# colinvaz/nmf-toolbox

Hardware: AMD Instinct MI355X
Metric: NMF multiplicative-update iterations/s (higher is better)
Workload: dtype f32; 1 GPU; nmf.m kl MU, V=16384x65536 K=256 fp32, V column-sharded over 1 GPU(s); m=16384, n=65536, K=256, T=1, divergence=kl

## Files before the change

### nmf_toolbox_amd/build.py

```python
from __future__ import annotations

import os
import subprocess
import sys
from concurrent.futures import ThreadPoolExecutor

HERE = os.path.dirname(os.path.abspath(__file__))
CSRC = os.path.join(HERE, "csrc")
INC = os.path.join(os.path.dirname(HERE), "include")
OUT = os.path.join(HERE, "libnmfx.so")
SOURCES = ["fused_cnmf_a.hip", "fused_cnmf_b.hip", "fused_cnmf_c.hip", "fused_cnmf_e.hip", "fused_cnmf_d.hip", "fused_cnmf_g.hip", "fused_cnmf_f.hip", "gemm_pipe_edge.hip", "gemm_pipe.hip", "gemm.hip", "fused_k224_256.hip", "fused_rag_k224_256.hip", "fused_k128_192.hip", "fused_rag_k128_192.hip", "fused_k32_96.hip", "fused_rag_k32_96.hip", "fused.hip", "aux.hip", "projfunc.hip", "small_mm.hip", "gemm64.hip", "engine.hip", "host_io.hip", "blocking.hip", "sc.hip", "sc64.hip", "multi_sc.hip", "rccl_backend.hip", "cmfwisa.hip", "seminmf.hip", "nmf64.hip", "nmf_batch.hip", "cnmf_batch.hip", "wnmf.hip", "wcnmf.hip"]
ARCH = "gfx950"


def _torch_lib_dir():
    try:
        import importlib.util
        spec = importlib.util.find_spec("torch")
        if spec and spec.origin:
            d = os.path.join(os.path.dirname(spec.origin), "lib")
            if os.path.exists(os.path.join(d, "libamdhip64.so")):
                return d
    except Exception:
        pass
    return None


def _deps(src, incdirs, seen=None):
    import re
    seen = set() if seen is None else seen
    if src in seen or not os.path.exists(src):
        return seen
    seen.add(src)
    with open(src) as f:
        for name in re.findall(r'^\s*#\s*include\s*"([^"]+)"', f.read(), re.M):
            for d in [os.path.dirname(src)] + incdirs:
                cand = os.path.join(d, name)
                if os.path.exists(cand):
                    _deps(cand, incdirs, seen)
                    break
    return seen


def _newer(src_list, target):
    if not os.path.exists(target):
        return True
    t = os.path.getmtime(target)
    return any(os.path.getmtime(s) > t for s in src_list)


VARIANTS = {
    "r5": ["-DNMFX_KL_MODE=0", "-DNMFX_G2_VEC=0", "-DNMFX_G1_ASM=0"],
    "kl1": ["-DNMFX_KL_MODE=1", "-DNMFX_G2_VEC=0", "-DNMFX_G1_ASM=0"],
    "kl2": ["-DNMFX_KL_MODE=2", "-DNMFX_G2_VEC=0", "-DNMFX_G1_ASM=0"],
    "kl2g2": ["-DNMFX_KL_MODE=2", "-DNMFX_G2_VEC=1", "-DNMFX_G1_ASM=0"],
}


def build(force: bool = False, verbose: bool = False, sanitize: bool = False, variant: str = "") -> str:
    srcs = [os.path.join(CSRC, s) for s in SOURCES if os.path.exists(os.path.join(CSRC, s))]
    objdir = os.path.join(CSRC, "_obj_asan" if sanitize else ("_obj_" + variant if variant else "_obj"))
    out = os.path.join(HERE, "libnmfx_asan.so") if sanitize else (os.path.join(HERE, "libnmfx_%s.so" % variant) if variant else OUT)
    vdefs = VARIANTS[variant] if variant else []
    san = ["-fsanitize=address,undefined", "-fno-sanitize=function", "-fno-gpu-sanitize", "-fno-sanitize-recover=undefined", "-Xarch_host", "-g", "-Xarch_host", "-fno-omit-frame-pointer"] if sanitize else []
    os.makedirs(objdir, exist_ok=True)
    hipcc = os.environ.get("HIPCC", "/opt/rocm/bin/hipcc")

    def compile_one(src):
        obj = os.path.join(objdir, os.path.basename(src) + ".o")
        if force or _newer(sorted(_deps(src, [CSRC, INC])) + [os.path.abspath(__file__)], obj):
            cmd = [hipcc, f"--offload-arch={ARCH}", "-O3", "-std=c++17", "-fPIC", "-Wall", "-Werror=uninitialized", "-Wno-pass-failed"] + san + vdefs + [
                   "-I", INC, "-I", CSRC, "-c", src, "-o", obj]
            if os.path.basename(src).startswith("fused_"):
                cmd[3:3] = ["-mllvm", "-pragma-unroll-threshold=1000000"]
            if verbose:
                print(" ".join(cmd), flush=True)
            subprocess.check_call(cmd)
        return obj

    with ThreadPoolExecutor(max_workers=min(len(srcs), 8)) as ex:
        objs = list(ex.map(compile_one, srcs))
    if force or _newer(objs, out):
        tl = _torch_lib_dir()
        libdirs = ([tl] if tl else []) + ["/opt/rocm/lib"]
        if sanitize:
            cmd = ["/opt/rocm/lib/llvm/bin/clang++", "-shared", "-fsanitize=address,undefined", "-fno-sanitize=function", "-o", out] + objs
        else:
            cmd = ["g++", "-shared", "-o", out] + objs
# ... 34 lines not shown
```

### nmf_toolbox_amd/csrc/fused.hip

```cpp
#include "nmfx_internal.h"

namespace nmfx {

bool fused_supported(int K) { return K >= 32 && K <= 256 && K % 32 == 0; }
bool fused_supported_T(int Kh, int T) {
    static const int ok[][2] = {{64, 8}, {64, 4}, {32, 8}, {32, 16}, {64, 2}, {32, 4}, {128, 2}, {128, 4},
                                {32, 3}, {32, 5}, {32, 6}, {64, 3}, {32, 10}, {32, 12}, {64, 5}, {64, 6},
                                {32, 7}, {32, 9}, {32, 11}, {64, 7}, {32, 13}, {32, 14}, {32, 15}, {128, 3}, {256, 2}};
    for (const auto &c : ok) if (c[0] == Kh && c[1] == T) return true;
    return false;
}

bool fused_supported_T_dual(int Kh, int T) { return fused_supported_T(Kh, T); }

#define NMFX_DECL(name) nmfx_status name(hipStream_t st, const FusedParams &p, int nsplit, bool d_rc, int func, bool do_g2, int epi)
NMFX_DECL(launch_fused_k32_96); NMFX_DECL(launch_fused_k128_192); NMFX_DECL(launch_fused_k224_256);
NMFX_DECL(launch_fused_rag_k32_96); NMFX_DECL(launch_fused_rag_k128_192); NMFX_DECL(launch_fused_rag_k224_256);
#undef NMFX_DECL
#define NMFX_DECL_T(name) nmfx_status name(hipStream_t st, const FusedParams &p, int nsplit, int func, bool do_g2)
NMFX_DECL_T(launch_fused_cnmf_a); NMFX_DECL_T(launch_fused_cnmf_b); NMFX_DECL_T(launch_fused_cnmf_c); NMFX_DECL_T(launch_fused_cnmf_d); NMFX_DECL_T(launch_fused_cnmf_e); NMFX_DECL_T(launch_fused_cnmf_f); NMFX_DECL_T(launch_fused_cnmf_g);
#undef NMFX_DECL_T

nmfx_status launch_fused(hipStream_t st, const FusedParams &p, int nsplit, bool d_rc, int func, bool do_g2, int epi) {
    constexpr int FT_ROWS = 128, FT_C = 64;
    if (p.R <= 0 || p.Cn <= 0 || p.c_per_split % FT_C || p.c_per_split <= 0 || nsplit < 1 || (long)(nsplit - 1) * p.c_per_split >= p.Cn) {
        set_error("launch_fused: bad split (R=%ld Cn=%ld c_per_split=%ld nsplit=%d)", p.R, p.Cn, p.c_per_split, nsplit);
        return NMFX_ERR_INVALID;
    }
    if (p.T > 1) {
        if (!d_rc || epi != 0 || p.K % p.T != 0 || !fused_supported_T(p.K / p.T, p.T)) {
            set_error("launch_fused: cnmf pass with (K = %d, T = %d) is not instantiated", p.K, p.T);
            return NMFX_ERR_UNSUPPORTED;
        }
        const int kh = p.K / p.T;
        if ((kh == 64 && (p.T == 8 || p.T == 4))) return launch_fused_cnmf_a(st, p, nsplit, func, do_g2);
        if (kh == 32 && (p.T == 8 || p.T == 16)) return launch_fused_cnmf_b(st, p, nsplit, func, do_g2);
        if ((kh == 32 && (p.T == 3 || p.T == 5 || p.T == 6)) || (kh == 64 && p.T == 3)) return launch_fused_cnmf_d(st, p, nsplit, func, do_g2);
        if ((kh == 32 && (p.T == 10 || p.T == 12)) || (kh == 64 && (p.T == 5 || p.T == 6))) return launch_fused_cnmf_e(st, p, nsplit, func, do_g2);
        if ((kh == 32 && (p.T == 7 || p.T == 9 || p.T == 11)) || (kh == 64 && p.T == 7)) return launch_fused_cnmf_f(st, p, nsplit, func, do_g2);
        if ((kh == 32 && (p.T == 13 || p.T == 14 || p.T == 15)) || (kh == 128 && p.T == 3) || (kh == 256 && p.T == 2)) return launch_fused_cnmf_g(st, p, nsplit, func, do_g2);
        return launch_fused_cnmf_c(st, p, nsplit, func, do_g2);
    }
    if (!fused_supported(p.K)) { set_error("launch_fused: K=%d not supported (multiples of 32 up to 256)", p.K); return NMFX_ERR_UNSUPPORTED; }
    if (d_rc && do_g2 && func == 0 && epi == 0 && p.os_k == 1 && p.os_r != 1 && NMFX_G2_VEC) epi = 2;
    const bool rag = p.R % FT_ROWS != 0 || p.Cn % FT_C != 0;
    if (p.K <= 96) return rag ? launch_fused_rag_k32_96(st, p, nsplit, d_rc, func, do_g2, epi) : launch_fused_k32_96(st, p, nsplit, d_rc, func, do_g2, epi);
    if (p.K <= 192) return rag ? launch_fused_rag_k128_192(st, p, nsplit, d_rc, func, do_g2, epi) : launch_fused_k128_192(st, p, nsplit, d_rc, func, do_g2, epi);
    return rag ? launch_fused_rag_k224_256(st, p, nsplit, d_rc, func, do_g2, epi) : launch_fused_k224_256(st, p, nsplit, d_rc, func, do_g2, epi);
}

}
```

### nmf_toolbox_amd/csrc/fused_kernel.h

```cpp
#pragma once
#include "nmfx_internal.h"

namespace nmfx {

typedef float f32x16 __attribute__((ext_vector_type(16)));
typedef float f32x2 __attribute__((ext_vector_type(2)));

typedef int i32x4 __attribute__((ext_vector_type(4)));

constexpr int FT_ROWS = 128;
constexpr int FT_C = 64;

__device__ __forceinline__ f32x2 pk_mul_t(f32x2 a, f32x2 b) { f32x2 d; asm("s_nop 0\n\tv_pk_mul_f32 %0, %1, %2" : "=v"(d) : "v"(a), "v"(b)); return d; }
__device__ __forceinline__ f32x2 pk_fma_t(f32x2 a, f32x2 b, f32x2 c) { f32x2 d; asm("s_nop 0\n\tv_pk_fma_f32 %0, %1, %2, %3" : "=v"(d) : "v"(a), "v"(b), "v"(c)); return d; }
__device__ __forceinline__ f32x2 pk_fnma(f32x2 a, f32x2 b, f32x2 c) { f32x2 d; asm("v_pk_fma_f32 %0, %1, %2, %3 neg_lo:[1,0,0] neg_hi:[1,0,0]" : "=v"(d) : "v"(a), "v"(b), "v"(c)); return d; }
__device__ __forceinline__ f32x2 pk_add(f32x2 a, f32x2 b) { f32x2 d; asm("v_pk_add_f32 %0, %1, %2" : "=v"(d) : "v"(a), "v"(b)); return d; }

__device__ __forceinline__ void mfma_settle_full(f32x16 &t) { asm volatile("s_nop 15\n\ts_nop 3" : "+v"(t)); }
__device__ __forceinline__ constexpr int rowmap(int reg, int h) { return (reg & 3) + 8 * (reg >> 2) + 4 * h; }
__device__ __forceinline__ i32x4 make_srd(const void *base, unsigned bytes) {
    const unsigned long long b = (unsigned long long)base;
    i32x4 s;
    s.x = (int)(unsigned)b;
    s.y = (int)((b >> 32) & 0xffffu);
    s.z = (int)bytes;
    s.w = 0x00020000;
    return s;
}

template <int K, bool D_RC, int FUNC, bool DO_G2, int EPI, bool RAG = false, int TT = 1>
__global__ __launch_bounds__(256, ((K <= 128 && FUNC != 4 && FUNC != 5) ? 2 : 1)) void fused_kernel(const FusedParams p) {
    extern __shared__ __attribute__((aligned(16))) float lds[];
    static_assert(TT == 1 || (D_RC && EPI == 0 && (K / TT) % 32 == 0 && K % TT == 0), "TT > 1: W-step form, K/TT a multiple of 32");
    if (p.run_if && *p.run_if == 0) return;
    constexpr int KH = K / TT;
    constexpr int LDY = KH + 4;
    constexpr int NKB = K / 32;
    constexpr int TROWS = FT_C + TT - 1;
    constexpr int BUF = TROWS * LDY;
    constexpr bool NEED_S = FUNC != 0;
    constexpr bool S_IN = FUNC == 7 || FUNC == 8 || FUNC == 10 || FUNC == 19 || FUNC == 20;
    constexpr int MF = FUNC == 8 ? 3 : ((FUNC == 10 || FUNC == 21) ? 1 : FUNC);
    static_assert(!S_IN || (!DO_G2 && D_RC && TT == 1), "partial-S passes: first product only, W-step form");
    constexpr bool DUAL = FUNC == 4 || FUNC == 5;
    constexpr bool NO_V = FUNC == 12 || FUNC == 14;
    constexpr int NVL = (!D_RC && !RAG) ? 8 : 32;
    constexpr bool SWAP = (!D_RC || EPI == 2) && NMFX_G2_VEC;
    static_assert(EPI != 2 || (D_RC && DO_G2 && FUNC == 0 && TT == 1), "EPI 2: W-step form, no first product");
    constexpr bool STB = FUNC == 15 || FUNC == 16;
    constexpr int EF = (FUNC == 15 || FUNC == 19) ? 11 : ((FUNC == 16 || FUNC == 20) ? 13 : FUNC);
    static_assert(!STB || (DO_G2 && D_RC && EPI == 0 && TT == 1), "functors 15 / 16: W-step form with the second product");
    constexpr bool ST2 = (EF == 11 || EF == 13) && !DO_G2 && D_RC;
    constexpr bool BQ = STB || ST2;
    constexpr bool EARLY = !DO_G2 && NEED_S;
    constexpr bool G1A = NMFX_G1_ASM;
    constexpr bool SADD = S_IN && G1A;
    constexpr bool PK = NMFX_KL_MODE == 2 && (MF == 2 || MF == 3) && !DUAL && EF == FUNC;
    constexpr int NU = (DUAL || EF == 11 || EF == 13) ? 8 : ((MF == 3 && NMFX_KL_MODE == 1) ? 6 : 4);
    static_assert(!DUAL || (K <= 192 && TT == 1), "dual-map kernels: K <= 192 (two accumulator sets + the stationary operand must fit 512 VGPRs: 501 at K = 192, spills at 224)");
    constexpr int NG = K / 8;
    constexpr int ROWS_PER_WAVE = (TROWS + 3) / 4;
    auto kofs = [](int kq) constexpr -> int { return (kq / KH) * LDY + (kq % KH); };
    constexpr int G2_KB = KH / 32, G2_NFULL = KH / 128, G2_WREM = G2_KB % 4;
    auto g2_kloc = [](int lb, int i) constexpr -> int {
        if (!NMFX_G2_VEC) return 32 * lb + i;
        return lb < 4 * G2_NFULL ? 128 * (lb / 4) + 4 * i + (lb % 4) : 128 * G2_NFULL + G2_WREM * i + (lb - 4 * G2_NFULL);
    };

    const int tid = threadIdx.x;
    const int lane = tid & 63;
    const int w = __builtin_amdgcn_readfirstlane(tid >> 6);
    const int l31 = lane & 31, h = lane >> 5;
    const long r_wg0 = (long)blockIdx.x * FT_ROWS;
    const long r0 = r_wg0 + 32 * w;
    const long r = r0 + l31;
    const long cbeg = (long)blockIdx.y * p.c_per_split;
    const long cend = cbeg + p.c_per_split < p.Cn ? cbeg + p.c_per_split : p.Cn;
    const int ntiles = RAG ? (int)((cend - cbeg + FT_C - 1) / FT_C) : (int)((cend - cbeg) / FT_C);
    const bool row_ok = !RAG || r < p.R;

    float xreg[NEED_S ? K / 2 : 1];
    if (NEED_S) {
#pragma unroll
        for (int s = 0; s < K / 2; ++s) {
            const int kq = 8 * (s >> 2) + (s & 3);
            xreg[s] = row_ok ? p.X[r * p.xs_r + (long)(kq % KH + 4 * h) * p.xs_k + (long)(TT - 1 - kq / KH) * p.xs_t] : 0.0f;
        }
// ... 17 lines not shown
    const unsigned y_voff = (unsigned)lane * 16u;
    auto dma_row = [&](const i32x4 ysrd, int b, int c) {
        const int row = w + 4 * c;
        if (TROWS % 4 != 0 && row >= TROWS) return;
        const unsigned dst = __builtin_amdgcn_readfirstlane(lds0 + (unsigned)((b * BUF + row * LDY) * 4));
        const unsigned soff = __builtin_amdgcn_readfirstlane((unsigned)(row * (TT > 1 ? KH : ystride) * 4));
        unsigned keep;
        if (lane < KH / 4)
            asm volatile("s_mov_b32 %0, m0\n\ts_mov_b32 m0, %3\n\ts_nop 0\n\tbuffer_load_dwordx4 %1, %2, %4 offen lds\n\ts_mov_b32 m0, %0"
                         : "=&s"(keep) : "v"(y_voff), "s"(ysrd), "s"(dst), "s"(soff) : "memory");
    };
    auto tile_rows = [&](int t) -> int {
        if (!RAG) return FT_C;
        const long left = cend - (cbeg + (long)t * FT_C);
        return left >= FT_C ? FT_C : (left > 0 ? (int)left : 0);
    };
    auto y_srd = [&](int t) {
        if (TT > 1) return make_srd(p.Y + (cbeg + (long)t * FT_C - (TT - 1)) * KH, (unsigned)((tile_rows(t) + TT - 1) * KH * 4));
        return make_srd(Yz + (cbeg + (long)t * FT_C) * ystride, (unsigned)(tile_rows(t) > 0 ? ((tile_rows(t) - 1) * ystride + K) * 4 : 0));
    };

    float d[32];
    const unsigned d_voff = D_RC ? (unsigned)((r + 4 * h * p.ldd) * 4) : (unsigned)((p.ldd * (r - r_wg0) + 4 * h) * 4);
    const long wg_rows = RAG ? (p.R - r_wg0 < FT_ROWS ? p.R - r_wg0 : (long)FT_ROWS) : (long)FT_ROWS;
    const __amdgpu_buffer_rsrc_t d_srd_fixed =
        __builtin_amdgcn_make_buffer_rsrc((void *)(p.D + p.ldd * r_wg0), 0, (int)(unsigned)(wg_rows * p.ldd * 4), 0x00020000);
    auto d_srd = [&](int t) {
        if (D_RC) return __builtin_amdgcn_make_buffer_rsrc((void *)(p.D + p.ldd * (cbeg + (long)t * FT_C)), 0, (int)(unsigned)(tile_rows(t) * p.ldd * 4), 0x00020000);
        return d_srd_fixed;
    };
    auto load_d_piece = [&](const __amdgpu_buffer_rsrc_t srd, int t, int i) {
        if (FUNC == 7 || NO_V) return;
        if (D_RC) {
#pragma unroll
            for (int u = 0; u < 2; ++u) {
                const int e = 2 * i + u, jb = e >> 4, reg = e & 15;
                const int soff = (int)(p.ldd * (32 * jb + (reg & 3) + 8 * (reg >> 2)) * 4);
                d[e] = __builtin_bit_cast(float, __builtin_amdgcn_raw_buffer_load_b32(srd, d_voff, soff, 0));
            }
        } else if ((i & 1) == 0) {
            const int f = i >> 1, jb = f >> 2, q = f & 3;
            const int soff = (int)((cbeg + (long)t * FT_C + 32 * jb + 8 * q) * 4);
            if (!RAG) {
                typedef unsigned u32x4 __attribute__((ext_vector_type(4)));
                typedef float f32x4 __attribute__((ext_vector_type(4)));
                const f32x4 q4 = __builtin_bit_cast(f32x4, (u32x4)__builtin_amdgcn_raw_buffer_load_b128(srd, d_voff, soff, 0));
                d[jb * 16 + 4 * q + 0] = q4.x; d[jb * 16 + 4 * q + 1] = q4.y; d[jb * 16 + 4 * q + 2] = q4.z; d[jb * 16 + 4 * q + 3] = q4.w;
                return;
            }
#pragma unroll
            for (int e = 0; e < 4; ++e)
                d[jb * 16 + 4 * q + e] = __builtin_bit_cast(float, __builtin_amdgcn_raw_buffer_load_b32(srd, d_voff, soff + 4 * e, 0));
        }
    };

    float sin_[S_IN ? 32 : 1];
    float sin_n[(S_IN && NMFX_G1_ASM) ? 32 : 1];
    auto s_srd = [&](int t) {
        return __builtin_amdgcn_make_buffer_rsrc((void *)(p.Sin ? p.Sin + p.ldd * (cbeg + (long)t * FT_C) : p.D), 0, p.Sin ? (int)(unsigned)(tile_rows(t) * p.ldd * 4) : 0, 0x00020000);
    };
    auto load_s_piece = [&](const __amdgpu_buffer_rsrc_t srd, int i, bool nxt = false) {
#pragma unroll
        for (int u = 0; u < 2; ++u) {
            const int e = 2 * i + u, jb = e >> 4, reg = e & 15;
            const float sv = __builtin_bit_cast(float, __builtin_amdgcn_raw_buffer_load_b32(srd, d_voff, (int)(p.ldd * (32 * jb + (reg & 3) + 8 * (reg >> 2)) * 4), 0));
            if (S_IN && NMFX_G1_ASM && nxt) sin_n[(S_IN && NMFX_G1_ASM) ? e : 0] = sv;
            else sin_[S_IN ? e : 0] = sv;
        }
    };

    double cost = 0.0;
    if (ntiles > 0) {
        const i32x4 ys = y_srd(0);
#pragma unroll
        for (int c = 0; c < ROWS_PER_WAVE; ++c) dma_row(ys, 0, c);
        const __amdgpu_buffer_rsrc_t ds0 = d_srd(0);
#pragma unroll
        for (int i = 0; i < 16; ++i) load_d_piece(ds0, 0, i);
        if (S_IN) {
            const __amdgpu_buffer_rsrc_t ss0 = s_srd(0);
#pragma unroll
            for (int i = 0; i < 16; ++i) load_s_piece(ss0, i);
        }
    }
    for (int t = 0; t < ntiles; ++t) {
        const int b = t & 1;
        const int tn = t + 1 < ntiles ? t + 1 : t;
        {
            if (EARLY || STB) { if (t == 0) asm volatile("s_waitcnt vmcnt(0)" ::: "memory"); }
            else if (NEED_S && !NO_V) {
                if (NVL == 32) asm volatile("s_waitcnt vmcnt(32)" ::: "memory");
                else asm volatile("s_waitcnt vmcnt(8)" ::: "memory");
            }
            else asm volatile("s_waitcnt vmcnt(0)" ::: "memory");
            __syncthreads();
        }
        const float *Yt = lds + b * BUF;
        const i32x4 ysn = y_srd(tn);
        const __amdgpu_buffer_rsrc_t dsn = d_srd(tn);
        const __amdgpu_buffer_rsrc_t ssn = S_IN ? s_srd(tn) : dsn;
        int dma_c = 0;
        auto dma_some = [&](int upto) {
#pragma unroll
            for (int c = 0; c < ROWS_PER_WAVE; ++c)
                if (c >= dma_c && c < upto) dma_row(ysn, b ^ 1, c);
            dma_c = upto > dma_c ? upto : dma_c;
        };

        f32x16 sacc[2];
        f32x16 sacc2[DUAL ? 2 : 1];
        float bq[BQ ? 2 : 1][BQ ? 16 : 1];
        const __amdgpu_buffer_rsrc_t rs_b = STB ? __builtin_amdgcn_make_buffer_rsrc((void *)(p.Rout + p.ldd * (cbeg + (long)t * FT_C)), 0, (int)(unsigned)(tile_rows(t) * p.ldd * 4), 0x00020000)
                                                : d_srd_fixed;
        float tc = 0.0f;
        float ts = 0.0f;
        f32x2 tc2[2] = {{0.0f, 0.0f}, {0.0f, 0.0f}}, ts2[2] = {{0.0f, 0.0f}, {0.0f, 0.0f}};
        f32x2 es2[2], er2[2], eq2[2];
        const int cvh = RAG ? tile_rows(t) - 4 * h : 0;
        float es[2], er[2], eq[2];
        auto emap_u = [&](int jb, int reg, int u) {
            const int sl = reg & 1;
            if (FUNC == 7) return;
            const float v = NO_V ? 0.0f : d[jb * 16 + reg];
            const bool live = !RAG || (32 * jb + (reg & 3) + 8 * (reg >> 2)) < cvh;
            if (FUNC == 4) {
                if (u == 0) { es[sl] = sacc[jb][reg]; er[sl] = __builtin_amdgcn_rcpf(es[sl]); }
                if (u == 1) eq[sl] = v * er[sl];
                if (u == 2) sacc2[jb][reg] = live ? er[sl] : 0.0f;
                if (u == 3) sacc[jb][reg] = live ? eq[sl] * er[sl] : 0.0f;
                if (u == 4) er[sl] = __builtin_amdgcn_logf(eq[sl]);
                if (u == 5) tc = live ? tc + eq[sl] : tc;
                if (u == 6) tc = live ? fmaf(-0.6931471805599453f, er[sl], tc) : tc;
                if (u == 5 || u == 6) asm volatile("" : "+v"(tc));
            } else if (FUNC == 5) {
                if (u == 0) { es[sl] = sacc[jb][reg]; er[sl] = __builtin_amdgcn_fmed3f(__builtin_amdgcn_logf(es[sl]), -3.0e38f, 3.0e38f); }
                if (u == 1) eq[sl] = ab_e1 * er[sl];
                if (u == 2) eq[sl] = __builtin_amdgcn_exp2f(eq[sl]);
                if (u == 3) er[sl] = __builtin_amdgcn_exp2f(ab_e2 * er[sl]);
// ... 78 lines not shown
                    sacc[jb][reg + 2 * pr + 1] = lv[2 * pr + 1] ? er2[pr].y : 0.0f;
                }
                if (MF == 3) {
                    eq2[0] = pk_fnma(er2[0], es2[0], es2[0]);
                    eq2[1] = pk_fnma(er2[1], es2[1], es2[1]);
                    er2[0].x = __builtin_amdgcn_logf(er2[0].x); er2[0].y = __builtin_amdgcn_logf(er2[0].y);
                }
            }
            if (b == 2 && MF == 3) {
                er2[1].x = __builtin_amdgcn_logf(er2[1].x); er2[1].y = __builtin_amdgcn_logf(er2[1].y);
#pragma unroll
                for (int pr = 0; pr < 2; ++pr) {
                    const f32x2 t = pk_fma_t(vv[pr], er2[pr], tc2[pr]);
                    const f32x2 u = pk_add(ts2[pr], eq2[pr]);
                    if (RAG) {
                        tc2[pr].x = lv[2 * pr] ? t.x : tc2[pr].x; tc2[pr].y = lv[2 * pr + 1] ? t.y : tc2[pr].y;
                        ts2[pr].x = lv[2 * pr] ? u.x : ts2[pr].x; ts2[pr].y = lv[2 * pr + 1] ? u.y : ts2[pr].y;
                    } else { tc2[pr] = t; ts2[pr] = u; }
                    asm volatile("" : "+v"(tc2[pr]), "+v"(ts2[pr]));
                }
            }
        };
        auto emap_fill = [&](int jb, int i, int M) {
            if (PK) {
#pragma unroll
                for (int q = 0; q < 4 * NBD; ++q)
                    if ((2 * q + 1) * M / (8 * NBD) == i) emap_burst(jb, q / NBD, q % NBD);
                return;
            }
            const int q0 = 16 * NU * i / M, q1 = 16 * NU * (i + 1) / M;
#pragma unroll
            for (int q = q0; q < q1; ++q) emap_u(jb, q / NU, q % NU);
        };
        auto g1_read = [&](int jb, int g) { return *reinterpret_cast<const float4 *>(Yt + (32 * jb + l31) * LDY + kofs(8 * g) + 4 * h); };
        if (NEED_S) {
#pragma unroll
            for (int jb = 0; jb < 2; ++jb)
#pragma unroll
                for (int e = 0; e < 16; ++e) sacc[jb][e] = (S_IN && !SADD) ? sin_[S_IN ? jb * 16 + e : 0] : 0.0f;
            float4 a_cur = g1_read(0, 0);
#pragma unroll
            for (int ph = 0; ph < 2; ++ph) {
#pragma unroll
                for (int g = 0; g < NG; ++g) {
                    float4 a_nxt = a_cur;
                    if (g + 1 < NG) a_nxt = g1_read(ph, g + 1);
                    else if (ph == 0) a_nxt = g1_read(1, 0);
                    auto one = [&](int e, float av) {
#if NMFX_G1_ASM
                      if (G1A) {
                        constexpr bool XA = K / 2 + (DO_G2 ? (DUAL ? 2 : 1) * NKB * 16 : 0) <= 256;
                        const bool first = g == 0 && e == 0 && (!S_IN || SADD);
                        if (ph == 1 && g == 0 && e == 0) {
                            if (XA) {
                                if (first) asm volatile("v_mfma_f32_32x32x2_f32 %0, %2, %3, 0\n\ts_nop 3" : "=&v"(sacc[1]), "+v"(sacc[0]) : "v"(av), "a"(xreg[0]));
                                else asm volatile("v_mfma_f32_32x32x2_f32 %0, %2, %3, %0\n\ts_nop 3" : "+v"(sacc[1]), "+v"(sacc[0]) : "v"(av), "a"(xreg[0]));
                            } else {
                                if (first) asm volatile("v_mfma_f32_32x32x2_f32 %0, %2, %3, 0\n\ts_nop 3" : "=&v"(sacc[1]), "+v"(sacc[0]) : "v"(av), "v"(xreg[0]));
                                else asm volatile("v_mfma_f32_32x32x2_f32 %0, %2, %3, %0\n\ts_nop 3" : "+v"(sacc[1]), "+v"(sacc[0]) : "v"(av), "v"(xreg[0]));
                            }
                            if (SADD) {
#pragma unroll
                                for (int q = 0; q < 16; ++q) sacc[0][q] += sin_[S_IN ? q : 0];
                            }
                        } else if (XA) {
                            if (first) asm volatile("v_mfma_f32_32x32x2_f32 %0, %1, %2, 0" : "=&v"(sacc[ph]) : "v"(av), "a"(xreg[4 * g + e]));
                            else asm volatile("v_mfma_f32_32x32x2_f32 %0, %1, %2, %0" : "+v"(sacc[ph]) : "v"(av), "a"(xreg[4 * g + e]));
                        } else {
                            if (first) asm volatile("v_mfma_f32_32x32x2_f32 %0, %1, %2, 0" : "=&v"(sacc[ph]) : "v"(av), "v"(xreg[4 * g + e]));
                            else asm volatile("v_mfma_f32_32x32x2_f32 %0, %1, %2, %0" : "+v"(sacc[ph]) : "v"(av), "v"(xreg[4 * g + e]));
                        }
                      } else
#endif
                        sacc[ph] = __builtin_amdgcn_mfma_f32_32x32x2f32(av, xreg[4 * g + e], sacc[ph], 0, 0, 0);
                        if (ph == 1) emap_fill(0, 4 * g + e, 4 * NG);
                        if (ph == 0 && e == 0) dma_some(((g + 1) * ROWS_PER_WAVE + NG - 1) / NG);
                        if (S_IN && ph == 1 && 4 * g + e < 16) load_s_piece(ssn, 4 * g + e, true);
                        __builtin_amdgcn_sched_barrier(0);
                    };
                    one(0, a_cur.x); one(1, a_cur.y); one(2, a_cur.z); one(3, a_cur.w);
                    a_cur = a_nxt;
                }
            }
        } else {
#pragma unroll
            for (int reg = 0; reg < 16; ++reg) emap_u(0, reg, 0);
#pragma unroll
            for (int reg = 0; reg < 16; ++reg) emap_u(1, reg, 0);
        }
#if NMFX_G1_ASM
        if (NEED_S && G1A && !DO_G2) {
            mfma_settle_full(sacc[1]);
            if (SADD) {
#pragma unroll
                for (int q = 0; q < 16; ++q) sacc[1][q] += sin_[S_IN ? 16 + q : 0];
            }
        }
#endif
        if (DO_G2) {
            if (STB) asm volatile("s_waitcnt vmcnt(0)" ::: "memory");
            auto g2_read = [&](int jb, int reg, float (&y)[NKB]) {
                if (NMFX_G2_VEC) {
                    const float *yrow = Yt + (32 * jb + rowmap(reg, h)) * LDY;
#pragma unroll
                    for (int pb = 0; pb < TT; ++pb) {
#pragma unroll
                        for (int c = 0; c < G2_NFULL; ++c) {
                            const float4 t4 = *reinterpret_cast<const float4 *>(yrow + pb * LDY + 128 * c + 4 * l31);
                            y[pb * G2_KB + 4 * c + 0] = t4.x; y[pb * G2_KB + 4 * c + 1] = t4.y; y[pb * G2_KB + 4 * c + 2] = t4.z; y[pb * G2_KB + 4 * c + 3] = t4.w;
                        }
                        if (G2_WREM == 2) {
                            const float2 t2 = *reinterpret_cast<const float2 *>(yrow + pb * LDY + 128 * G2_NFULL + 2 * l31);
                            y[pb * G2_KB + 4 * G2_NFULL + 0] = t2.x; y[pb * G2_KB + 4 * G2_NFULL + 1] = t2.y;
                        } else {
#pragma unroll
                            for (int j = 0; j < G2_WREM; ++j) y[pb * G2_KB + 4 * G2_NFULL + j] = yrow[pb * LDY + 128 * G2_NFULL + G2_WREM * l31 + j];
                        }
                    }
                    return;
                }
                const float *yrow = Yt + (32 * jb + rowmap(reg, h)) * LDY + l31;
#pragma unroll
                for (int kb = 0; kb < NKB; ++kb) y[kb] = yrow[kofs(32 * kb)];
            };
            float y_cur[NKB], y_nxt[NKB];
            g2_read(0, 0, y_cur);
#pragma unroll
            for (int st = 0; st < 32; ++st) {
                const int jb = st >> 4, reg = st & 15;
                if (st + 1 < 32) g2_read((st + 1) >> 4, (st + 1) & 15, y_nxt);
                const float rr = sacc[jb][reg];
                const float rr2 = DUAL ? sacc2[jb][reg] : 0.0f;
#pragma unroll
                for (int kb = 0; kb < NKB; ++kb) {
#if NMFX_G1_ASM
                    if (NEED_S && G1A && st == 0 && kb == 0) {
                        if (SWAP) asm volatile("v_mfma_f32_32x32x2_f32 %0, %2, %3, %0\n\ts_nop 3" : "+a"(acc[0]), "+v"(sacc[1]) : "v"(rr), "v"(y_cur[0]));
                        else asm volatile("v_mfma_f32_32x32x2_f32 %0, %2, %3, %0\n\ts_nop 3" : "+a"(acc[0]), "+v"(sacc[1]) : "v"(y_cur[0]), "v"(rr));
                    } else
#endif
                    acc[kb] = SWAP ? __builtin_amdgcn_mfma_f32_32x32x2f32(rr, y_cur[kb], acc[kb], 0, 0, 0) : __builtin_amdgcn_mfma_f32_32x32x2f32(y_cur[kb], rr, acc[kb], 0, 0, 0);
                    if (jb == 0 && NEED_S) emap_fill(1, (reg * NKB + kb) * (DUAL ? 2 : 1), 16 * NKB * (DUAL ? 2 : 1));
                    if (kb == 0 && !NEED_S) dma_some((st + 1) * ROWS_PER_WAVE / 24 < ROWS_PER_WAVE ? (st + 1) * ROWS_PER_WAVE / 24 : ROWS_PER_WAVE);
                    if (kb == NKB / 2 && jb == (NEED_S ? 1 : 0)) load_d_piece(dsn, tn, reg);
                    if (STB && kb == 1 && (jb == 1 || reg >= 8)) {
                        auto put = [&](int j2, int r2) {
                            const float bv = bq[STB ? j2 : 0][STB ? r2 : 0];
                            if (row_ok) __builtin_amdgcn_raw_buffer_store_b32(__builtin_bit_cast(unsigned, bv), rs_b, d_voff, (int)(p.ldd * (32 * j2 + (r2 & 3) + 8 * (r2 >> 2)) * 4), 0);
                        };
                        if (jb == 0) { put(0, 2 * (reg - 8)); put(0, 2 * (reg - 8) + 1); }
                        else put(1, reg);
                    }
                    __builtin_amdgcn_sched_barrier(0);
                    if (DUAL) {
                        acc2[kb] = SWAP ? __builtin_amdgcn_mfma_f32_32x32x2f32(rr2, y_cur[kb], acc2[kb], 0, 0, 0) : __builtin_amdgcn_mfma_f32_32x32x2f32(y_cur[kb], rr2, acc2[kb], 0, 0, 0);
                        if (jb == 0) emap_fill(1, (reg * NKB + kb) * 2 + 1, 32 * NKB);
                        __builtin_amdgcn_sched_barrier(0);
                    }
                }
#pragma unroll
                for (int kb = 0; kb < NKB; ++kb) y_cur[kb] = y_nxt[kb];
            }
        } else {
            if (S_IN) asm volatile("s_waitcnt vmcnt(32)" ::: "memory");
            else if (EARLY) asm volatile("s_waitcnt vmcnt(0)" ::: "memory");
            if (PK) {
#pragma unroll
                for (int q = 0; q < 4 * NBD; ++q) emap_burst(1, q / NBD, q % NBD);
            } else {
#pragma unroll
                for (int reg = 0; reg < 16; ++reg)
#pragma unroll
                    for (int u = 0; u < NU; ++u) emap_u(1, reg, u);
            }
            if (D_RC && ((MF >= 2 && MF <= 3) || FUNC == 7 || FUNC == 1 || FUNC == 21 || ST2) && p.Rout) {
                const __amdgpu_buffer_rsrc_t rs = __builtin_amdgcn_make_buffer_rsrc((void *)(p.Rout + p.ldd * (cbeg + (long)t * FT_C)), 0, (int)(unsigned)(tile_rows(t) * p.ldd * 4), 0x00020000);
                if (row_ok) {
#pragma unroll
                    for (int e = 0; e < 32; ++e) {
                        const int jb = e >> 4, reg = e & 15;
                        const float rv = sacc[jb][reg];
                        __builtin_amdgcn_raw_buffer_store_b32(__builtin_bit_cast(unsigned, rv), rs, d_voff, (int)(p.ldd * (32 * jb + (reg & 3) + 8 * (reg >> 2)) * 4), 0);
                    }
                }
            }
            if (ST2 && p.Rout2) {
                const __amdgpu_buffer_rsrc_t rs2 = __builtin_amdgcn_make_buffer_rsrc((void *)(p.Rout2 + p.ldd * (cbeg + (long)t * FT_C)), 0, (int)(unsigned)(tile_rows(t) * p.ldd * 4), 0x00020000);
                if (row_ok) {
#pragma unroll
                    for (int e = 0; e < 32; ++e) {
                        const int jb = e >> 4, reg = e & 15;
                        const float bv = bq[BQ ? jb : 0][BQ ? reg : 0];
                        __builtin_amdgcn_raw_buffer_store_b32(__builtin_bit_cast(unsigned, bv), rs2, d_voff, (int)(p.ldd * (32 * jb + (reg & 3) + 8 * (reg >> 2)) * 4), 0);
                    }
                }
            }
#pragma unroll
            for (int i = 0; i < 16; ++i) load_d_piece(dsn, tn, i);
        }
        dma_some(ROWS_PER_WAVE);
        if (SADD) {
#pragma unroll
            for (int e = 0; e < 32; ++e) sin_[S_IN ? e : 0] = sin_n[(S_IN && NMFX_G1_ASM) ? e : 0];
        }
        if (MF == 3 && NMFX_KL_MODE == 2) cost += row_ok ? ((double)tc2[0].x + (double)tc2[0].y + (double)tc2[1].x + (double)tc2[1].y) * 0.6931471805599453 + ((double)ts2[0].x + (double)ts2[0].y + (double)ts2[1].x + (double)ts2[1].y) : 0.0;
        else if (MF == 3 && NMFX_KL_MODE == 1) cost += row_ok ? (double)tc * 0.6931471805599453 + (double)ts : 0.0;
        else cost += row_ok ? (double)tc : 0.0;
    }

    auto e_kloc = [&](int kb, int reg) -> int { return g2_kloc(kb % G2_KB, SWAP ? l31 : rowmap(reg, h)); };
    auto e_row = [&](int reg) -> long { return SWAP ? r0 + rowmap(reg, h) : r; };
    auto e_ok = [&](int reg) -> bool { return !RAG || e_row(reg) < p.R; };
    if (DO_G2) {
        if (EPI == 0 || EPI == 2) {
            float *out = p.out + (long)blockIdx.y * p.slab_stride + (TT == 1 ? (long)blockIdx.z * p.oz_stride : 0L);
#pragma unroll
            for (int q = 0; q < 16 * NKB; ++q) {
                const int kb = SWAP ? q % NKB : q / 16, reg = SWAP ? q / NKB : q % 16;
                if (e_ok(reg)) {
                    const long oi = e_row(reg) * p.os_r + (long)e_kloc(kb, reg) * p.os_k + (long)(TT - 1 - kb / G2_KB) * p.os_t;
                    out[oi] = acc[kb][reg];
                    if (DUAL) p.out2[(long)blockIdx.y * p.slab_stride + oi] = acc2[kb][reg];
                }
            }
        } else {
            bool lines_done = false;
            if (SWAP && !DUAL && G2_NFULL > 0 && p.H64 && !p.fix && !p.sqrt_rule) {
                lines_done = true;
#pragma unroll
                for (int reg = 0; reg < 16; ++reg) {
                    if (!e_ok(reg)) continue;
#pragma unroll
                    for (int c = 0; c < G2_NFULL; ++c) {
                        const int k0 = 128 * c + 4 * l31;
                        const long idx0 = (long)k0 + (long)K * e_row(reg);
                        double hv[4], dn[4];
#pragma unroll
                        for (int o = 0; o < 4; ++o) hv[o] = p.H64[idx0 + o];
#pragma unroll
                        for (int o = 0; o < 4; ++o) dn[o] = (p.den ? (double)p.den[idx0 + o] : p.denvec[k0 + o]) + (p.lam ? (double)p.lam[k0 + o] : 0.0);
#pragma unroll
                        for (int o = 0; o < 4; ++o) hv[o] = hv[o] * ((double)acc[4 * c + o][reg] / fmax(dn[o], 2.220446049250313e-16));
// ... 53 lines not shown
```

### nmf_toolbox_amd/csrc/nmfx_internal.h

```cpp
#pragma once
#include <hip/hip_runtime.h>
#include <stddef.h>
#include <stdint.h>

#include "nmfx.h"

#define NMFX_EPS_F 2.220446049250313e-16f

namespace nmfx {

void set_error(const char *fmt, ...);
#define NMFX_HIP(call)                                                                    \
    do {                                                                                  \
        hipError_t e_ = (call);                                                           \
        if (e_ != hipSuccess) {                                                           \
            nmfx::set_error("%s failed: %s (%s:%d)", #call, hipGetErrorString(e_), __FILE__, __LINE__); \
            return NMFX_ERR_HIP;                                                          \
        }                                                                                 \
    } while (0)

#define TRY(x) do { nmfx_status s_ = (x); if (s_ != NMFX_OK) return s_; } while (0)

struct LdsAttrOnce {
    int set_bytes[64] = {};
// ... 63 lines not shown
    int clamp0;
    int store_c;
    int epi;
    int cost_div;
    float cost_alpha, cost_beta;
    const float *Vref;
    long ldv;
    double *cost_partials;
    long cost_ncols;
    int splitk;
    long slab_stride;
    long kc_per_split;
    int zbatch;
    long zA_off, zB_off;
    int zB_lim, zB_tstride;
};
bool gemm_pipe_eligible(const GemmParams &p);

nmfx_status launch_gemm(hipStream_t st, const GemmParams &p, long *blocks_out = nullptr);
nmfx_status gemm_auto(hipStream_t st, GemmParams p, void *scratch, size_t scratch_bytes);
int gemm_pick_split(long M, long N, long Kc);
long gemm_grid_blocks(long M, long N);
size_t gemm_scratch_bytes(long M, long N, long Kc);

#ifndef NMFX_KL_MODE
#define NMFX_KL_MODE 2
#endif
#ifndef NMFX_G2_VEC
#define NMFX_G2_VEC 1
#endif
#ifndef NMFX_G1_ASM
#define NMFX_G1_ASM 1
#endif
constexpr bool KL_CONSISTENT_COST = NMFX_KL_MODE != 0;
struct FusedParams {
    const float *X;
    long xs_r, xs_k;
    int T;
    long xs_t, os_t;
    const float *Y;
    long y_stride;
    int nz;
    long yz_stride, oz_stride;
    const float *D;
    long ldd;
    long R, Cn;
    long c_per_split;
    int K;
    float *out;
    float *Rout2;
    float *Rout;
    const float *Sin;
    float *out2;
    float ab_alpha, ab_beta;
    float inv_exp;
    long slab_stride, os_r, os_k;
    double *cost_partials;
    float *Hio;
    const float *den;
    const double *denvec;
    const float *lam;
    const uint8_t *fix;
    int sqrt_rule;
    double *H64;
    const int *run_if;
};
bool fused_supported(int K);
bool fused_supported_T_dual(int Kh, int T);
bool fused_supported_T(int Kh, int T);
nmfx_status launch_fused(hipStream_t st, const FusedParams &p, int nsplit, bool d_rc, int func, bool do_g2, int epi);

bool h_update_gram_supported(int K);
nmfx_status h_update_gram(hipStream_t st, float *H, const float *G, const float *Gn, int n_slabs, long slab_stride, int K, long n, const float *lam,
                          const uint8_t *fix, double *H64 = nullptr);

nmfx_status reduce_slabs(hipStream_t st, const float *slabs, int nslab, long slab_stride, long count, float *out,
                         int accumulate);
nmfx_status col_reduce(hipStream_t st, const float *X, long rows, long ld, int ncols, int mode, double *out);
nmfx_status row_reduce(hipStream_t st, const float *X, int rows, long ld, long ncols, int mode, double *out, void *scratch);
size_t row_reduce_scratch_bytes(int rows);
struct WUpdateParams {
    float *W;
    const float *N;
    const float *P;
    const double *Pvec;
    const float *Pvecf;
    const float *lamW;
    const uint8_t *fixW;
    long m;
    int K, T;
    double *sumsq;
    float inv_exp;
    int rule;
    int n_chunks;
    int fuse_norm;
    double *colsum_out;
    double *dndp;
    int stats_only;
// ... 95 lines not shown
```

Measured before the change: 65.94 iterations/s.

## Restructure fused tile loop seam to overlap next-tile barrier, loads and cost fold

Removes the tile-top vmcnt wait and __syncthreads in the fused KL kernel. They are replaced by a carried first G1 operand, a barrier placed after the first MFMA, and a mid-G2 wait-plus-barrier, so the tile boundary overlaps with compute. With SEAM=3 (the default), it also prefetches the first G2 operand and the next-tile buffer descriptors early, and splits the double-precision cost accumulation into stages interleaved with the G2 MFMAs. It adds optional s_memtime instrumentation (off by default) and new build variants. The risk is subtle synchronisation hazards around the LDS double buffer and extra register pressure.

```diff
diff --git a/nmf_toolbox_amd/build.py b/nmf_toolbox_amd/build.py
--- a/nmf_toolbox_amd/build.py
+++ b/nmf_toolbox_amd/build.py
@@ -54,6 +54,10 @@
     "kl1": ["-DNMFX_KL_MODE=1", "-DNMFX_G2_VEC=0", "-DNMFX_G1_ASM=0"],
     "kl2": ["-DNMFX_KL_MODE=2", "-DNMFX_G2_VEC=0", "-DNMFX_G1_ASM=0"],
     "kl2g2": ["-DNMFX_KL_MODE=2", "-DNMFX_G2_VEC=1", "-DNMFX_G1_ASM=0"],
+    "noseam": ["-DNMFX_SEAM=0"],
+    "seamb": ["-DNMFX_SEAM=1"],
+    "stamps": ["-DNMFX_STAMPS=1"],
+    "stamps_noseam": ["-DNMFX_STAMPS=1", "-DNMFX_SEAM=0"],
 }
 
 
diff --git a/nmf_toolbox_amd/csrc/fused.hip b/nmf_toolbox_amd/csrc/fused.hip
--- a/nmf_toolbox_amd/csrc/fused.hip
+++ b/nmf_toolbox_amd/csrc/fused.hip
@@ -21,8 +21,28 @@
 NMFX_DECL_T(launch_fused_cnmf_a); NMFX_DECL_T(launch_fused_cnmf_b); NMFX_DECL_T(launch_fused_cnmf_c); NMFX_DECL_T(launch_fused_cnmf_d); NMFX_DECL_T(launch_fused_cnmf_e); NMFX_DECL_T(launch_fused_cnmf_f); NMFX_DECL_T(launch_fused_cnmf_g);
 #undef NMFX_DECL_T
 
-nmfx_status launch_fused(hipStream_t st, const FusedParams &p, int nsplit, bool d_rc, int func, bool do_g2, int epi) {
+#if NMFX_STAMPS
+static unsigned long long *stamps_buf() {
+    static unsigned long long *buf = nullptr;
+    if (!buf && (hipMalloc(&buf, 32 * sizeof(unsigned long long)) != hipSuccess || hipMemset(buf, 0, 32 * sizeof(unsigned long long)) != hipSuccess)) buf = nullptr;
+    return buf;
+}
+extern "C" __attribute__((visibility("default"))) int nmfx_stamps_read(unsigned long long *out, int reset) {
+    unsigned long long *buf = stamps_buf();
+    if (!buf || hipDeviceSynchronize() != hipSuccess || hipMemcpy(out, buf, 32 * sizeof(unsigned long long), hipMemcpyDeviceToHost) != hipSuccess) return 1;
+    if (reset && hipMemset(buf, 0, 32 * sizeof(unsigned long long)) != hipSuccess) return 1;
+    return 0;
+}
+#endif
+
+nmfx_status launch_fused(hipStream_t st, const FusedParams &p_in, int nsplit, bool d_rc, int func, bool do_g2, int epi) {
     constexpr int FT_ROWS = 128, FT_C = 64;
+#if NMFX_STAMPS
+    FusedParams p = p_in;
+    p.stamps = stamps_buf();
+#else
+    const FusedParams &p = p_in;
+#endif
     if (p.R <= 0 || p.Cn <= 0 || p.c_per_split % FT_C || p.c_per_split <= 0 || nsplit < 1 || (long)(nsplit - 1) * p.c_per_split >= p.Cn) {
         set_error("launch_fused: bad split (R=%ld Cn=%ld c_per_split=%ld nsplit=%d)", p.R, p.Cn, p.c_per_split, nsplit);
         return NMFX_ERR_INVALID;
diff --git a/nmf_toolbox_amd/csrc/fused_kernel.h b/nmf_toolbox_amd/csrc/fused_kernel.h
--- a/nmf_toolbox_amd/csrc/fused_kernel.h
+++ b/nmf_toolbox_amd/csrc/fused_kernel.h
@@ -44,7 +44,8 @@
     static_assert(!S_IN || (!DO_G2 && D_RC && TT == 1), "partial-S passes: first product only, W-step form");
     constexpr bool DUAL = FUNC == 4 || FUNC == 5;
     constexpr bool NO_V = FUNC == 12 || FUNC == 14;
-    constexpr int NVL = (!D_RC && !RAG) ? 8 : 32;
+    constexpr int VLW = (!D_RC && !RAG) ? 4 : 1;
+    constexpr int NVL = 32 / VLW;
     constexpr bool SWAP = (!D_RC || EPI == 2) && NMFX_G2_VEC;
     static_assert(EPI != 2 || (D_RC && DO_G2 && FUNC == 0 && TT == 1), "EPI 2: W-step form, no first product");
     constexpr bool STB = FUNC == 15 || FUNC == 16;
@@ -53,6 +54,8 @@
     constexpr bool ST2 = (EF == 11 || EF == 13) && !DO_G2 && D_RC;
     constexpr bool BQ = STB || ST2;
     constexpr bool EARLY = !DO_G2 && NEED_S;
+    constexpr bool SEAM_B = (NMFX_SEAM & 1) && DO_G2 && NEED_S && !DUAL && !STB && !S_IN && TT == 1;
+    constexpr bool SEAM_C = SEAM_B && (NMFX_SEAM & 2);
     constexpr bool G1A = NMFX_G1_ASM;
     constexpr bool SADD = S_IN && G1A;
     constexpr bool PK = NMFX_KL_MODE == 2 && (MF == 2 || MF == 3) && !DUAL && EF == FUNC;
@@ -136,6 +139,7 @@
     auto load_d_piece = [&](const __amdgpu_buffer_rsrc_t srd, int t, int i) {
         if (FUNC == 7 || NO_V) return;
         if (D_RC) {
+            static_assert(!D_RC || VLW == 1, "W-step form: 16 pieces of two dword loads");
 #pragma unroll
             for (int u = 0; u < 2; ++u) {
                 const int e = 2 * i + u, jb = e >> 4, reg = e & 15;
@@ -145,7 +149,7 @@
         } else if ((i & 1) == 0) {
             const int f = i >> 1, jb = f >> 2, q = f & 3;
             const int soff = (int)((cbeg + (long)t * FT_C + 32 * jb + 8 * q) * 4);
-            if (!RAG) {
+            if (VLW == 4) {
                 typedef unsigned u32x4 __attribute__((ext_vector_type(4)));
                 typedef float f32x4 __attribute__((ext_vector_type(4)));
                 const f32x4 q4 = __builtin_bit_cast(f32x4, (u32x4)__builtin_amdgcn_raw_buffer_load_b128(srd, d_voff, soff, 0));
@@ -187,27 +191,55 @@
             for (int i = 0; i < 16; ++i) load_s_piece(ss0, i);
         }
     }
+    auto g1_first = [&](const float *Yb) { return *reinterpret_cast<const float4 *>(Yb + l31 * LDY + 4 * h); };
+    float4 a_carry = {0.0f, 0.0f, 0.0f, 0.0f};
+    if (SEAM_B && ntiles > 0) {
+        asm volatile("s_waitcnt vmcnt(%0)\n\ts_barrier" :: "n"(NO_V ? 0 : NVL) : "memory");
+        a_carry = g1_first(lds);
+    }
+#if NMFX_STAMPS
+    constexpr bool STAMPED = DO_G2 && NEED_S && !DUAL && !STB && !S_IN && TT == 1;
+    unsigned long long st_sum[8] = {0, 0, 0, 0, 0, 0, 0, 0}, st_prev = 0;
+    auto stamp = [&](int seg) {
+        if (!STAMPED) return;
+        __builtin_amdgcn_sched_barrier(0);
+        unsigned long long tk;
+        asm volatile("s_memtime %0\n\ts_waitcnt lgkmcnt(0)" : "=s"(tk) :: "memory");
+        __builtin_amdgcn_sched_barrier(0);
+        if (seg >= 0) st_sum[seg] += tk - st_prev;
+        st_prev = tk;
+    };
+    stamp(-1);
+#define NMFX_STAMP(seg) stamp(seg)
+#else
+#define NMFX_STAMP(seg) ((void)0)
+#endif
     for (int t = 0; t < ntiles; ++t) {
         const int b = t & 1;
         const int tn = t + 1 < ntiles ? t + 1 : t;
-        {
+        if (!SEAM_B) {
             if (EARLY || STB) { if (t == 0) asm volatile("s_waitcnt vmcnt(0)" ::: "memory"); }
             else if (NEED_S && !NO_V) {
+                static_assert(NVL == 32 / VLW && (NVL == 32 || NVL == 8), "the tile-top wait counts the V-load instructions load_d_piece issues");
                 if (NVL == 32) asm volatile("s_waitcnt vmcnt(32)" ::: "memory");
                 else asm volatile("s_waitcnt vmcnt(8)" ::: "memory");
             }
             else asm volatile("s_waitcnt vmcnt(0)" ::: "memory");
+            NMFX_STAMP(0);
             __syncthreads();
-        }
+            NMFX_STAMP(1);
+        } else { NMFX_STAMP(0); NMFX_STAMP(1); }
         const float *Yt = lds + b * BUF;
         const i32x4 ysn = y_srd(tn);
         const __amdgpu_buffer_rsrc_t dsn = d_srd(tn);
+        i32x4 ysn_y = {0, 0, 0, 0};
+        __amdgpu_buffer_rsrc_t dsn_y = d_srd_fixed;
         const __amdgpu_buffer_rsrc_t ssn = S_IN ? s_srd(tn) : dsn;
         int dma_c = 0;
         auto dma_some = [&](int upto) {
 #pragma unroll
             for (int c = 0; c < ROWS_PER_WAVE; ++c)
-                if (c >= dma_c && c < upto) dma_row(ysn, b ^ 1, c);
+                if (c >= dma_c && c < upto) dma_row(SEAM_C ? ysn_y : ysn, b ^ 1, c);
             dma_c = upto > dma_c ? upto : dma_c;
         };
 
@@ -352,13 +384,54 @@
 #pragma unroll
             for (int q = q0; q < q1; ++q) emap_u(jb, q / NU, q % NU);
         };
+        constexpr bool CF_PK = MF == 3 && NMFX_KL_MODE == 2;
+        constexpr int CF_STAGES = CF_PK ? 5 : 1;
+        double cf_c[4], cf_s[4], cf_cs = 0.0, cf_ss = 0.0;
+        auto cost_fold = [&](int s) {
+            if (s >= 0 && CF_PK) {
+                if (s == 0) { cf_c[0] = (double)tc2[0].x; cf_c[1] = (double)tc2[0].y; cf_c[2] = (double)tc2[1].x; cf_c[3] = (double)tc2[1].y; asm volatile("" : "+v"(cf_c[0]), "+v"(cf_c[1]), "+v"(cf_c[2]), "+v"(cf_c[3])); }
+                if (s == 1) { cf_cs = cf_c[0] + cf_c[1] + cf_c[2] + cf_c[3]; asm volatile("" : "+v"(cf_cs)); }
+                if (s == 2) { cf_s[0] = (double)ts2[0].x; cf_s[1] = (double)ts2[0].y; cf_s[2] = (double)ts2[1].x; cf_s[3] = (double)ts2[1].y; asm volatile("" : "+v"(cf_s[0]), "+v"(cf_s[1]), "+v"(cf_s[2]), "+v"(cf_s[3])); }
+                if (s == 3) { cf_ss = cf_s[0] + cf_s[1] + cf_s[2] + cf_s[3]; asm volatile("" : "+v"(cf_ss)); }
+                if (s == 4) { cost += row_ok ? cf_cs * 0.6931471805599453 + cf_ss : 0.0; asm volatile("" : "+v"(cost)); }
+            } else if (s <= 0) {
+                if (MF == 3 && NMFX_KL_MODE == 2) cost += row_ok ? ((double)tc2[0].x + (double)tc2[0].y + (double)tc2[1].x + (double)tc2[1].y) * 0.6931471805599453 + ((double)ts2[0].x + (double)ts2[0].y + (double)ts2[1].x + (double)ts2[1].y) : 0.0;
+                else if (MF == 3 && NMFX_KL_MODE == 1) cost += row_ok ? (double)tc * 0.6931471805599453 + (double)ts : 0.0;
+                else cost += row_ok ? (double)tc : 0.0;
+            }
+        };
+        auto g2_read = [&](int jb, int reg, float (&y)[NKB]) {
+            if (NMFX_G2_VEC) {
+                const float *yrow = Yt + (32 * jb + rowmap(reg, h)) * LDY;
+#pragma unroll
+                for (int pb = 0; pb < TT; ++pb) {
+#pragma unroll
+                    for (int c = 0; c < G2_NFULL; ++c) {
+                        const float4 t4 = *reinterpret_cast<const float4 *>(yrow + pb * LDY + 128 * c + 4 * l31);
+                        y[pb * G2_KB + 4 * c + 0] = t4.x; y[pb * G2_KB + 4 * c + 1] = t4.y; y[pb * G2_KB + 4 * c + 2] = t4.z; y[pb * G2_KB + 4 * c + 3] = t4.w;
+                    }
+                    if (G2_WREM == 2) {
+                        const float2 t2 = *reinterpret_cast<const float2 *>(yrow + pb * LDY + 128 * G2_NFULL + 2 * l31);
+                        y[pb * G2_KB + 4 * G2_NFULL + 0] = t2.x; y[pb * G2_KB + 4 * G2_NFULL + 1] = t2.y;
+                    } else {
+#pragma unroll
+                        for (int j = 0; j < G2_WREM; ++j) y[pb * G2_KB + 4 * G2_NFULL + j] = yrow[pb * LDY + 128 * G2_NFULL + G2_WREM * l31 + j];
+                    }
+                }
+                return;
+            }
+            const float *yrow = Yt + (32 * jb + rowmap(reg, h)) * LDY + l31;
+#pragma unroll
+            for (int kb = 0; kb < NKB; ++kb) y[kb] = yrow[kofs(32 * kb)];
+        };
+        float y_cur[NKB], y_nxt[NKB];
         auto g1_read = [&](int jb, int g) { return *reinterpret_cast<const float4 *>(Yt + (32 * jb + l31) * LDY + kofs(8 * g) + 4 * h); };
         if (NEED_S) {
 #pragma unroll
             for (int jb = 0; jb < 2; ++jb)
 #pragma unroll
                 for (int e = 0; e < 16; ++e) sacc[jb][e] = (S_IN && !SADD) ? sin_[S_IN ? jb * 16 + e : 0] : 0.0f;
-            float4 a_cur = g1_read(0, 0);
+            float4 a_cur = SEAM_B ? a_carry : g1_read(0, 0);
 #pragma unroll
             for (int ph = 0; ph < 2; ++ph) {
 #pragma unroll
@@ -366,6 +439,7 @@
                     float4 a_nxt = a_cur;
                     if (g + 1 < NG) a_nxt = g1_read(ph, g + 1);
                     else if (ph == 0) a_nxt = g1_read(1, 0);
+                    else if (SEAM_C) g2_read(0, 0, y_cur);
                     auto one = [&](int e, float av) {
 #if NMFX_G1_ASM
                       if (G1A) {
@@ -393,6 +467,17 @@
                       } else
 #endif
                         sacc[ph] = __builtin_amdgcn_mfma_f32_32x32x2f32(av, xreg[4 * g + e], sacc[ph], 0, 0, 0);
+                        if (ph == 0 && g == 0 && e == 0) NMFX_STAMP(2);
+                        if (g == NG - 1 && e == 3) NMFX_STAMP(3 + ph);
+                        if (SEAM_B && ph == 0 && g == 0 && e == 0) {
+                            asm volatile("s_barrier" ::: "memory");
+                            if (SEAM_C) {
+                                int tq = tn;
+                                asm volatile("" : "+s"(tq));
+                                ysn_y = y_srd(tq);
+                                dsn_y = d_srd(tq);
+                            }
+                        }
                         if (ph == 1) emap_fill(0, 4 * g + e, 4 * NG);
                         if (ph == 0 && e == 0) dma_some(((g + 1) * ROWS_PER_WAVE + NG - 1) / NG);
                         if (S_IN && ph == 1 && 4 * g + e < 16) load_s_piece(ssn, 4 * g + e, true);
@@ -419,36 +504,12 @@
 #endif
         if (DO_G2) {
             if (STB) asm volatile("s_waitcnt vmcnt(0)" ::: "memory");
-            auto g2_read = [&](int jb, int reg, float (&y)[NKB]) {
-                if (NMFX_G2_VEC) {
-                    const float *yrow = Yt + (32 * jb + rowmap(reg, h)) * LDY;
-#pragma unroll
-                    for (int pb = 0; pb < TT; ++pb) {
-#pragma unroll
-                        for (int c = 0; c < G2_NFULL; ++c) {
-                            const float4 t4 = *reinterpret_cast<const float4 *>(yrow + pb * LDY + 128 * c + 4 * l31);
-                            y[pb * G2_KB + 4 * c + 0] = t4.x; y[pb * G2_KB + 4 * c + 1] = t4.y; y[pb * G2_KB + 4 * c + 2] = t4.z; y[pb * G2_KB + 4 * c + 3] = t4.w;
-                        }
-                        if (G2_WREM == 2) {
-                            const float2 t2 = *reinterpret_cast<const float2 *>(yrow + pb * LDY + 128 * G2_NFULL + 2 * l31);
-                            y[pb * G2_KB + 4 * G2_NFULL + 0] = t2.x; y[pb * G2_KB + 4 * G2_NFULL + 1] = t2.y;
-                        } else {
-#pragma unroll
-                            for (int j = 0; j < G2_WREM; ++j) y[pb * G2_KB + 4 * G2_NFULL + j] = yrow[pb * LDY + 128 * G2_NFULL + G2_WREM * l31 + j];
-                        }
-                    }
-                    return;
-                }
-                const float *yrow = Yt + (32 * jb + rowmap(reg, h)) * LDY + l31;
-#pragma unroll
-                for (int kb = 0; kb < NKB; ++kb) y[kb] = yrow[kofs(32 * kb)];
-            };
-            float y_cur[NKB], y_nxt[NKB];
-            g2_read(0, 0, y_cur);
+            if (!SEAM_C) g2_read(0, 0, y_cur);
 #pragma unroll
             for (int st = 0; st < 32; ++st) {
                 const int jb = st >> 4, reg = st & 15;
                 if (st + 1 < 32) g2_read((st + 1) >> 4, (st + 1) & 15, y_nxt);
+                else if (SEAM_B) a_carry = g1_first(lds + (b ^ 1) * BUF);
                 const float rr = sacc[jb][reg];
                 const float rr2 = DUAL ? sacc2[jb][reg] : 0.0f;
 #pragma unroll
@@ -460,9 +521,13 @@
                     } else
 #endif
                     acc[kb] = SWAP ? __builtin_amdgcn_mfma_f32_32x32x2f32(rr, y_cur[kb], acc[kb], 0, 0, 0) : __builtin_amdgcn_mfma_f32_32x32x2f32(y_cur[kb], rr, acc[kb], 0, 0, 0);
+                    if (NEED_S && st == 0 && kb == 0) NMFX_STAMP(5);
+                    if (NEED_S && reg == 15 && kb == NKB - 1) NMFX_STAMP(6 + jb);
                     if (jb == 0 && NEED_S) emap_fill(1, (reg * NKB + kb) * (DUAL ? 2 : 1), 16 * NKB * (DUAL ? 2 : 1));
                     if (kb == 0 && !NEED_S) dma_some((st + 1) * ROWS_PER_WAVE / 24 < ROWS_PER_WAVE ? (st + 1) * ROWS_PER_WAVE / 24 : ROWS_PER_WAVE);
-                    if (kb == NKB / 2 && jb == (NEED_S ? 1 : 0)) load_d_piece(dsn, tn, reg);
+                    if (SEAM_B && st == 16 && kb == 0) asm volatile("s_waitcnt vmcnt(0)\n\ts_barrier" ::: "memory");
+                    if (SEAM_C && jb == 1 && kb == 0 && reg >= 1 && reg <= CF_STAGES) cost_fold(reg - 1);
+                    if (kb == NKB / 2 && jb == (NEED_S ? 1 : 0)) load_d_piece(SEAM_C ? dsn_y : dsn, tn, reg);
                     if (STB && kb == 1 && (jb == 1 || reg >= 8)) {
                         auto put = [&](int j2, int r2) {
                             const float bv = bq[STB ? j2 : 0][STB ? r2 : 0];
@@ -523,11 +588,18 @@
 #pragma unroll
             for (int e = 0; e < 32; ++e) sin_[S_IN ? e : 0] = sin_n[(S_IN && NMFX_G1_ASM) ? e : 0];
         }
-        if (MF == 3 && NMFX_KL_MODE == 2) cost += row_ok ? ((double)tc2[0].x + (double)tc2[0].y + (double)tc2[1].x + (double)tc2[1].y) * 0.6931471805599453 + ((double)ts2[0].x + (double)ts2[0].y + (double)ts2[1].x + (double)ts2[1].y) : 0.0;
-        else if (MF == 3 && NMFX_KL_MODE == 1) cost += row_ok ? (double)tc * 0.6931471805599453 + (double)ts : 0.0;
-        else cost += row_ok ? (double)tc : 0.0;
+        if (!SEAM_C) cost_fold(-1);
     }
 
+#if NMFX_STAMPS
+    if (STAMPED && p.stamps && lane == 0) {
+        unsigned long long *dst = p.stamps + (D_RC ? 0 : 16);
+#pragma unroll
+        for (int i = 0; i < 8; ++i) atomicAdd(dst + i, st_sum[i]);
+        atomicAdd(dst + 8, (unsigned long long)ntiles);
+    }
+#endif
+#undef NMFX_STAMP
     auto e_kloc = [&](int kb, int reg) -> int { return g2_kloc(kb % G2_KB, SWAP ? l31 : rowmap(reg, h)); };
     auto e_row = [&](int reg) -> long { return SWAP ? r0 + rowmap(reg, h) : r; };
     auto e_ok = [&](int reg) -> bool { return !RAG || e_row(reg) < p.R; };
diff --git a/nmf_toolbox_amd/csrc/nmfx_internal.h b/nmf_toolbox_amd/csrc/nmfx_internal.h
--- a/nmf_toolbox_amd/csrc/nmfx_internal.h
+++ b/nmf_toolbox_amd/csrc/nmfx_internal.h
@@ -119,7 +119,13 @@
 #ifndef NMFX_G1_ASM
 #define NMFX_G1_ASM 1
 #endif
-constexpr bool KL_CONSISTENT_COST = NMFX_KL_MODE != 0;
+#ifndef NMFX_SEAM
+#define NMFX_SEAM 3
+#endif
+#ifndef NMFX_STAMPS
+#define NMFX_STAMPS 0
+#endif
+constexpr bool KL_CONSISTENT_COST =NMFX_KL_MODE != 0;
 struct FusedParams {
     const float *X;
     long xs_r, xs_k;
@@ -151,6 +157,9 @@
     int sqrt_rule;
     double *H64;
     const int *run_if;
+#if NMFX_STAMPS
+    unsigned long long *stamps;
+#endif
 };
 bool fused_supported(int K);
 bool fused_supported_T_dual(int Kh, int T);
```

Result: no change. 66.15 iterations/s, median of 6 (+0.3%).
